# rare-resilience-ai/Osteosarcoma_DiffusionModel

Measured on AMD Instinct MI355X. Metric: synthetic patients/sec (full T-step reverse sample), higher is better.
Workload: dtype f32; 1 GPU; reverse sampling of conditional patients, T=1000, D=2000 (50 mut + 1900 expr + 50 pathway), hidden [256,512,256], 3 scenario conditions (BASELINE config 3); patients_per_gpu=100000, T=1000, parallelism=patients sharded over 1 GPU(s), no collective, sampler=chain, chunk_rows=65536, streams=2, graph=True

## Files before the change

osteosarcoma_diffusionmodel_amd/csrc/chain.h:

```cpp
#pragma once
#include "gemm_glds.h"
#include "epilogues.h"
#include "xpose.h"
#include "launch.h"

namespace osd {

constexpr int CHAIN_MAX_LAYERS = 24;
enum : int { CK_INPUT = 0, CK_GN32 = 1, CK_GN64 = 2, CK_POST = 3 };
enum : unsigned { CHAIN_OK = 0, CHAIN_TIMEOUT = 1, CHAIN_ABORT = 2 };

struct ChainLayer {
  const float* A; int lda;
  int K, K0;
  int F;
  int in0, ld0, in1, ld1;
  int out, ldo;
  int kind;
  const float* bias; const float* gamma; const float* beta;
};

struct ChainArgs {
  ChainLayer L[CHAIN_MAX_LAYERS];
  int n_layers;
  float* ws; long long ws_stride;
  float* x; int D;
  int n, n_tiles;
  int t_first, n_steps;
  unsigned base_done;
  const float* cproj; int ldc;
  const float* temb; int ldt;
  const float* coef;
  const float* z; int ldzz; long long z_step_stride; int z_t_first;
  uint64_t seed; uint32_t row_offset;
  float* mut_mask; int mutation_dim;
  unsigned* progress;
  unsigned* status;
  unsigned* queue;
  unsigned* cu_arrivals;
  int stagger;
  unsigned long long spin_budget;
  unsigned long long* stamps;
};

typedef __attribute__((address_space(1))) unsigned gu32;

__device__ __forceinline__ unsigned ld_relaxed_agent(const unsigned* p) {
  return __hip_atomic_load(p, __ATOMIC_RELAXED, __HIP_MEMORY_SCOPE_AGENT);
}
__device__ __forceinline__ void st_relaxed_agent(unsigned* p, unsigned v) {
  __hip_atomic_store(p, v, __ATOMIC_RELAXED, __HIP_MEMORY_SCOPE_AGENT);
}

__device__ __forceinline__ bool chain_wait(const unsigned* word, unsigned want, unsigned* status, unsigned long long budget, int lane) {
  if ((unsigned)__builtin_amdgcn_readfirstlane((int)ld_relaxed_agent(word)) >= want) return true;
  const unsigned long long t0 = __builtin_amdgcn_s_memrealtime();
  for (;;) {
    __builtin_amdgcn_s_sleep(32);
    if ((unsigned)__builtin_amdgcn_readfirstlane((int)ld_relaxed_agent(word)) >= want) return true;
    if ((unsigned)__builtin_amdgcn_readfirstlane((int)ld_relaxed_agent(status)) != CHAIN_OK) return false;
    if (__builtin_amdgcn_s_memrealtime() - t0 > budget) {
      if (lane == 0) st_relaxed_agent(status, CHAIN_TIMEOUT);
      return false;
    }
  }
}

constexpr int CHAIN_PRM_FLOATS = 512;

template <int NPB>
struct XposeRowsOut {
  const WaveXpose<NPB>& xp; float* out; int ldo;
  __device__ __forceinline__ void put(int fb, int pb, int q, int l31, int h, float4 v) const { (void)fb; xp.put(pb, q, l31, h, v); }
  __device__ __forceinline__ void flush(int fb, int lane) const { xp.template store_rows<false>(out + 32 * fb, ldo, lane, 0, 0); }
};
template <int NPB>
struct XposeRowsIn {
  const WaveXpose<NPB>& xp; const float* src; int ld;
  __device__ __forceinline__ void load(int fb, int lane) const { xp.template load_rows<false>(src + 32 * fb, ld, lane, 0, 0); }
  __device__ __forceinline__ float4 get(int fb, int pb, int q, int l31, int h) const { (void)fb; return xp.get(pb, q, l31, h); }
};

template <int GW, int NFB, int NPB, int PS, class Out>
__device__ __forceinline__ void chain_gn_silu(f32x16 (&acc)[NFB][NPB], const float* __restrict__ prm, int fl, const Out& o, int lane,
                                              unsigned long long* ts = nullptr) {
  static_assert(GW >= 8 && NFB * 32 >= GW, "wave must own whole groups");
  constexpr int RPG = GW / 2;
  constexpr int NG = NFB * 16 / RPG;
  const int l31 = lane & 31, h = lane >> 5;
#pragma unroll
  for (int fb = 0; fb < NFB; ++fb)
#pragma unroll
    for (int q = 0; q < 4; ++q) {
      const float4 bv = *reinterpret_cast<const float4*>(prm + fl + 32 * fb + 8 * q + 4 * h);
#pragma unroll
      for (int pb = 0; pb < NPB; ++pb) {
        acc[fb][pb][4 * q] += bv.x; acc[fb][pb][4 * q + 1] += bv.y;
        acc[fb][pb][4 * q + 2] += bv.z; acc[fb][pb][4 * q + 3] += bv.w;
      }
    }
  if (ts) { asm volatile("s_waitcnt vmcnt(0) lgkmcnt(0)" ::: "memory"); ts[0] = __builtin_amdgcn_s_memtime(); }
  float mean[NPB][NG], rstd[NPB][NG];
#pragma unroll
  for (int pb = 0; pb < NPB; ++pb)
#pragma unroll
    for (int g = 0; g < NG; ++g) {
      float s = 0.f;
#pragma unroll
      for (int j = 0; j < RPG; ++j) { const int Li = g * RPG + j; s += acc[Li / 16][pb][Li % 16]; }
      s += swap_halves(s);
      const float m = s * (1.0f / GW);
      float qs = 0.f;
#pragma unroll
      for (int j = 0; j < RPG; ++j) { const int Li = g * RPG + j; const float d = acc[Li / 16][pb][Li % 16] - m; qs = fmaf(d, d, qs); }
      qs += swap_halves(qs);
      mean[pb][g] = m;
      rstd[pb][g] = 1.0f / sqrtf(qs * (1.0f / GW) + GN_EPS);
    }
  if (ts) { asm volatile("s_nop 0" ::: "memory"); ts[1] = __builtin_amdgcn_s_memtime(); ts[2] = ts[1]; }
#pragma unroll
  for (int fb = 0; fb < NFB; ++fb) {
#pragma unroll
    for (int q = 0; q < 4; ++q) {
      const int f = fl + 32 * fb + 8 * q + 4 * h;
      const float4 gv = *reinterpret_cast<const float4*>(prm + PS + f);
      const float4 bev = *reinterpret_cast<const float4*>(prm + 2 * PS + f);
      const int g = (fb * 16 + 4 * q) / RPG;
#pragma unroll
      for (int pb = 0; pb < NPB; ++pb) {
        const float m = mean[pb][g], r = rstd[pb][g];
        float4 y;
        y.x = silu_f(fmaf((acc[fb][pb][4 * q] - m) * r, gv.x, bev.x));
        y.y = silu_f(fmaf((acc[fb][pb][4 * q + 1] - m) * r, gv.y, bev.y));
        y.z = silu_f(fmaf((acc[fb][pb][4 * q + 2] - m) * r, gv.z, bev.z));
        y.w = silu_f(fmaf((acc[fb][pb][4 * q + 3] - m) * r, gv.w, bev.w));
        o.put(fb, pb, q, l31, h, y);
      }
    }
    o.flush(fb, lane);
  }
}

template <int NFB, int NPB, int PS, class In, class Out>
__device__ __forceinline__ void chain_input(f32x16 (&acc)[NFB][NPB], const float* __restrict__ prm, int fl, const In& in, const Out& o, int lane) {
  const int l31 = lane & 31, h = lane >> 5;
#pragma unroll
  for (int fb = 0; fb < NFB; ++fb) {
    in.load(fb, lane);
#pragma unroll
    for (int q = 0; q < 4; ++q) {
      const int f = fl + 32 * fb + 8 * q + 4 * h;
      const float4 bv = *reinterpret_cast<const float4*>(prm + f);
      const float4 tv = *reinterpret_cast<const float4*>(prm + PS + f);
#pragma unroll
      for (int pb = 0; pb < NPB; ++pb) {
        const float4 cv = in.get(fb, pb, q, l31, h);
        float4 v;
        v.x = ((acc[fb][pb][4 * q] + bv.x) + tv.x) + cv.x;
        v.y = ((acc[fb][pb][4 * q + 1] + bv.y) + tv.y) + cv.y;
        v.z = ((acc[fb][pb][4 * q + 2] + bv.z) + tv.z) + cv.z;
        v.w = ((acc[fb][pb][4 * q + 3] + bv.w) + tv.w) + cv.w;
        o.put(fb, pb, q, l31, h, v);
      }
    }
    o.flush(fb, lane);
  }
}

#ifndef OSD_EXP
#define OSD_EXP 0
#endif
template <int NFB, int NPB, bool PRE = false, bool GUARD = true>
__device__ __forceinline__ void chain_posterior(f32x16 (&acc)[NFB][NPB], const float* __restrict__ prm, int fl, float* __restrict__ x, int ldx,
                                                int prow, int pcol, float cA, float cB, float cC, int t, const float* __restrict__ zrow, int ldzz,
                                                uint64_t seed, uint32_t row_id0, int f_glob, float* __restrict__ mut_mask, int mutation_dim,
                                                const WaveXpose<NPB>& xp, int lane, float4 (*pre)[4 * NPB] = nullptr) {
  const int l31 = lane & 31, h = lane >> 5;
  if (prow <= 0) return;
  const bool do_mask = t == 0 && mut_mask != nullptr;
#pragma unroll
  for (int fb = 0; fb < NFB; ++fb) {
    const int cols = pcol - 32 * fb;
    if (GUARD && cols <= 0) break;
    if constexpr (PRE) {
      if (!(OSD_EXP & 2)) {
        xp.commit_rows(*pre, lane);
        if (fb + 1 < NFB && cols - 32 > 0) xp.template issue_rows<GUARD>(*pre, x + 32 * (fb + 1), ldx, lane, prow, cols - 32);
      }
    } else {
      xp.template load_rows<GUARD>(x + 32 * fb, ldx, lane, prow, cols);
    }
#pragma unroll
    for (int pb = 0; pb < NPB; ++pb) {
      const int p = 32 * pb + l31;
      const int pc = (!GUARD || p < prow) ? p : prow - 1;
#pragma unroll
      for (int q = 0; q < 4; ++q) {
        const int fo = 32 * fb + 8 * q + 4 * h;
        const float4 bv = *reinterpret_cast<const float4*>(prm + fl + fo);
        const float e[4] = {acc[fb][pb][4 * q] + bv.x, acc[fb][pb][4 * q + 1] + bv.y, acc[fb][pb][4 * q + 2] + bv.z, acc[fb][pb][4 * q + 3] + bv.w};
        const float4 xq = xp.get(pb, q, l31, h);
        const float xv[4] = {xq.x, xq.y, xq.z, xq.w};
        float4 zz = make_float4(0.f, 0.f, 0.f, 0.f);
        if (t > 0 && cC != 0.f) {
          if (zrow) {
            const int fc = (!GUARD || fo < pcol - 4) ? fo : pcol - 4;
            zz = ldg4(zrow + (size_t)pc * ldzz + fc);
          } else if (!(OSD_EXP & 1)) {
            zz = randn4(seed, row_id0 + (uint32_t)p, (uint32_t)((f_glob + fo) >> 2), (uint32_t)t, TAG_POSTERIOR);
          }
        }
        const float zv[4] = {zz.x, zz.y, zz.z, zz.w};
        float o[4];
#pragma unroll
        for (int r = 0; r < 4; ++r) o[r] = fmaf(cA, xv[r], fmaf(cB, e[r], cC * zv[r]));
        if (do_mask && p < prow && fo < pcol && f_glob + fo < mutation_dim) {
          float* mrow = mut_mask + (size_t)p * mutation_dim;
#pragma unroll
          for (int r = 0; r < 4; ++r)
            if (f_glob + fo + r < mutation_dim) stg1(mrow + f_glob + fo + r, (o[r] > 0.5f) ? 1.0f : 0.0f);
        }
        xp.put(pb, q, l31, h, make_float4(o[0], o[1], o[2], o[3]));
      }
    }
    if (!(OSD_EXP & 4)) xp.template store_rows<GUARD>(x + 32 * fb, ldx, lane, prow, cols);
  }
}

#ifndef CHAIN_EPI_PRIO
#define CHAIN_EPI_PRIO 0
#endif
#ifndef CHAIN_BP
#define CHAIN_BP 128
#endif
#if CHAIN_BP == 128
typedef Tile<128, 128, 64, 64> ChainTile;
constexpr int CHAIN_WPS = 2;
#else
typedef Tile<128, 64, 64, 32> ChainTile;
constexpr int CHAIN_WPS = 3;
#endif
#ifdef OSD_DIAG
constexpr int CHAIN_KCNT = 12;
constexpr int CHAIN_STAMP_FLOATS = 2 * 4 * CHAIN_KCNT;
#else
constexpr int CHAIN_KCNT = 10;
constexpr int CHAIN_STAMP_FLOATS = 80;
#endif
constexpr int CHAIN_PRM_OFF = 2 * (ChainTile::BF * BK + ChainTile::BP * BK) + 4 + CHAIN_STAMP_FLOATS;
constexpr int CHAIN_LDS_BYTES = (CHAIN_PRM_OFF + 2 * CHAIN_PRM_FLOATS) * 4;
static_assert(CHAIN_PRM_OFF % 4 == 0, "parameter blocks are read as float4");

template <bool STAMP>
__global__ __launch_bounds__(NTHREADS, CHAIN_WPS) void chain_kernel(const ChainArgs* __restrict__ gp) {
  const ChainArgs& a = *gp;
  typedef ChainTile T;
  typedef GldsTile<T> G;
  static_assert(T::BF == 128 && T::BP % 32 == 0, "staging below assumes a 128-row weight image");
  constexpr int NW = NTHREADS / 64;
  constexpr int NPW = 16 / NW;
  constexpr int NPWB = T::BP / 8 / NW;
  constexpr int PROWS = 8 * NW;
  constexpr unsigned PBYTES = 1024u * NW;
  extern __shared__ __attribute__((aligned(16))) float smem[];
  float* As0 = smem;
  float* As1 = smem + G::A_ELEMS;
  float* Bs0 = smem + 2 * G::A_ELEMS;
  float* Bs1 = smem + 2 * G::A_ELEMS + G::B_ELEMS;
  volatile int& s_flag = *reinterpret_cast<volatile int*>(smem + 2 * (G::A_ELEMS + G::B_ELEMS));

  const int tid = threadIdx.x;
  const int lane = tid & 63;
  const int wave = __builtin_amdgcn_readfirstlane(tid >> 6);
  const int wf = (wave / T::NWP) * T::WF;
  const int wp = (wave % T::NWP) * T::WP;

  float* const ws = a.ws + (long long)blockIdx.x * a.ws_stride;
  WaveXpose<T::NPB> xp;
  {
    const int xo = wave * (T::NPB * 1024);
    xp.buf = xo < G::A_ELEMS ? As1 + xo : Bs1 + (xo - G::A_ELEMS);
  }
  float* const prm_base = smem + CHAIN_PRM_OFF;
  int pcur = 0;

  if (a.cu_arrivals && a.stagger > 0) {
    if (wave == 0) {
      const unsigned hw = __builtin_amdgcn_s_getreg(0xF804);
      const unsigned xcc = __builtin_amdgcn_s_getreg(0xF814) & 7;
      const unsigned key = (xcc << 8) | ((hw >> 8) & 0xFF);
      unsigned r = 0;
      if (lane == 0) r = atomicAdd(a.cu_arrivals + key, 1u);
      s_flag = __builtin_amdgcn_readfirstlane((int)(r & 1u));
    }
    __syncthreads();
    const int late = __builtin_amdgcn_readfirstlane(s_flag);
    __syncthreads();
    if (late) {
      const unsigned long long t0 = __builtin_amdgcn_s_memtime();
      while (__builtin_amdgcn_s_memtime() - t0 < (unsigned long long)a.stagger) __builtin_amdgcn_s_sleep(16);
    }
  }

  unsigned long long c_dep = 0, c_pro = 0, c_k = 0, c_epi = 0, c_units = 0;
  unsigned long long* const kcnt = reinterpret_cast<unsigned long long*>(smem + 2 * (G::A_ELEMS + G::B_ELEMS) + 4);
  if constexpr (STAMP) {
    if (tid < 4 * CHAIN_KCNT) kcnt[tid] = 0;
    __syncthreads();
  }
  const unsigned long long c_start = STAMP ? __builtin_amdgcn_s_memtime() : 0;
  const long long n_units = (long long)a.n_tiles * a.n_steps;
  int c_iter = 0;
  (void)c_iter;
  for (;;) {
    const unsigned long long td0 = STAMP ? __builtin_amdgcn_s_memtime() : 0;
#ifdef CHAIN_STATIC_UNITS
    static_assert(true, "");
    const long long u = (long long)blockIdx.x + (long long)c_iter * gridDim.x;
    ++c_iter;
#else
    if (wave == 0) {
      unsigned nu = 0;
      if (lane == 0) nu = atomicAdd(a.queue, 1u);
      s_flag = __builtin_amdgcn_readfirstlane((int)nu);
    }
    __syncthreads();
    const long long u = (unsigned)__builtin_amdgcn_readfirstlane(s_flag);
    __syncthreads();
#endif
    if (u >= n_units) break;
    const int tile = (int)(u % a.n_tiles);
    const int si = (int)(u / a.n_tiles);
    const int t = a.t_first - si;
    const int p0 = tile * T::BP;
    const int P = (a.n - p0 < T::BP) ? a.n - p0 : T::BP;

    if (wave == 0) {
      bool ok = (unsigned)__builtin_amdgcn_readfirstlane((int)ld_relaxed_agent(a.status)) == CHAIN_OK;
      if (ok && si > 0) {
        ok = chain_wait(a.progress + tile, a.base_done + (unsigned)si, a.status, a.spin_budget, lane);
        if (ok) __builtin_amdgcn_fence(__ATOMIC_ACQUIRE, "agent");
      }
      s_flag = ok ? 1 : 0;
      asm volatile("s_waitcnt vmcnt(0) lgkmcnt(0)" ::: "memory");
    }
    __syncthreads();
    const int go = __builtin_amdgcn_readfirstlane(s_flag);
    if (!go) return;
    if constexpr (STAMP) { c_dep += __builtin_amdgcn_s_memtime() - td0; ++c_units; }

    auto first_stage = [&](const ChainLayer& Lr, int f0n, bool do_a, bool do_b, int pb) {
      struct { const float* A; int lda, F, in0, ld0, K0, K; } Ln{Lr.A, Lr.lda, Lr.F, Lr.in0, Lr.ld0, Lr.K0, Lr.K};
      if (do_a && wave < 2) {
        const int kind = Lr.kind;
        const float* src = Lr.bias;
        if (wave == 1) src = Lr.beta;
        else if (lane >= 32) src = kind == CK_INPUT ? a.temb + (size_t)t * a.ldt : (kind == CK_POST ? Lr.bias : Lr.gamma);
        if (wave == 0 || (kind != CK_INPUT && kind != CK_POST)) {
          int f = f0n + 4 * (lane & 31);
          f = f < Ln.F - 4 ? f : Ln.F - 4;
          glds16(src + f, __builtin_amdgcn_readfirstlane(lds_addr(prm_base + pb * CHAIN_PRM_FLOATS) + (unsigned)wave * 1024u));
        }
      }
      const float* const xrows = a.x + (size_t)p0 * a.D;
      int ln = lane;
      asm volatile("" : "+v"(ln));
      const int r0 = wave * 8 + (ln >> 3);
      const int k4 = 4 * ((ln & 7) ^ ((r0 >> 1) & 7));
      const unsigned la = __builtin_amdgcn_readfirstlane(lds_addr(As0) + (unsigned)wave * 1024u);
      const unsigned lb = __builtin_amdgcn_readfirstlane(lds_addr(Bs0) + (unsigned)wave * 1024u);
      if (do_a) {
#pragma unroll
        for (int j = 0; j < NPW; ++j) {
          int rg = f0n + r0 + PROWS * j;
          rg = rg < Ln.F ? rg : Ln.F - 1;
          glds16(Ln.A + (size_t)rg * Ln.lda + k4, __builtin_amdgcn_readfirstlane(la + (unsigned)j * PBYTES));
        }
      }
      if (do_b) {
        const bool from_x = Ln.in0 < 0;
        const float* bb = from_x ? xrows : ws + Ln.in0;
        const int rows = from_x ? P : T::BP;
        const int kend = Ln.K0 < Ln.K ? Ln.K0 : Ln.K;
        const int k = k4 < kend - 4 ? k4 : kend - 4;
#pragma unroll
        for (int j = 0; j < NPWB; ++j) {
          int rg = r0 + PROWS * j;
          rg = rg < rows ? rg : rows - 1;
          glds16(bb + (size_t)rg * Ln.ld0 + k, __builtin_amdgcn_readfirstlane(lb + (unsigned)j * PBYTES));
        }
      }
    };
    unsigned long long tt0 = STAMP ? __builtin_amdgcn_s_memtime() : 0;
    first_stage(a.L[0], 0, true, true, pcur);
    asm volatile("s_waitcnt vmcnt(0)" ::: "memory");
    __syncthreads();

    for (int l = 0; l < a.n_layers; ++l) {
      const ChainLayer& L = a.L[l];
      const gfloat_ptr LA = uniform_ptr(L.A);
      const int Llda = L.lda, LK0 = L.K0, Lld0 = L.ld0, Lld1 = L.ld1;
      const int F = L.F, K = L.K;
      const float* const B0g = (L.in0 < 0) ? a.x + (size_t)p0 * a.D : ws + L.in0;
      const float* const B1g = ws + L.in1;
      const gfloat_ptr B0 = uniform_ptr(B0g), B1 = uniform_ptr(B1g);
      const int rowsB = (L.in0 < 0) ? P : T::BP;
      const int nk = (K + BK - 1) / BK;
      const int nft = (F + T::BF - 1) / T::BF;
      for (int ft = 0; ft < nft; ++ft) {
        const int f0 = ft * T::BF;
        int ln = lane;
        asm volatile("" : "+v"(ln));
        const int l31 = ln & 31, h = ln >> 5;
        int st_row[NPW], st_k4[NPW];
#pragma unroll
        for (int j = 0; j < NPW; ++j) {
          st_row[j] = (j * NW + wave) * 8 + (ln >> 3);
          st_k4[j] = 4 * ((ln & 7) ^ ((st_row[j] >> 1) & 7));
        }
        int a_rd[T::NFB], a_sw[T::NFB], b_rd[T::NPB], b_sw[T::NPB];
#pragma unroll
        for (int fb = 0; fb < T::NFB; ++fb) { const int R = wf + 32 * fb + l31; a_rd[fb] = R * BK; a_sw[fb] = h ^ ((R >> 1) & 7); }
#pragma unroll
        for (int pb = 0; pb < T::NPB; ++pb) { const int R = wp + 32 * pb + l31; b_rd[pb] = R * BK; b_sw[pb] = h ^ ((R >> 1) & 7); }
        unsigned offA[NPW], offB[NPWB];
#pragma unroll
        for (int j = 0; j < NPW; ++j) {
          int rg = f0 + st_row[j];
          rg = rg < F ? rg : F - 1;
          offA[j] = (unsigned)(rg * Llda + st_k4[j]) * 4u;
        }
#pragma unroll
        for (int j = 0; j < NPWB; ++j) {
          int rb = st_row[j];
          rb = rb < rowsB ? rb : rowsB - 1;
          offB[j] = (unsigned)(rb * Lld0 + st_k4[j]) * 4u;
        }
        int b_panel = 0;
        auto b_offsets_for = [&](int k0) {
          const int want = k0 < LK0 ? 0 : 1;
          if (want != b_panel) {
            b_panel = want;
            const int ld = want ? Lld1 : Lld0;
#pragma unroll
            for (int j = 0; j < NPWB; ++j) {
              int rb = st_row[j];
              rb = rb < rowsB ? rb : rowsB - 1;
              offB[j] = (unsigned)(rb * ld + st_k4[j]) * 4u;
            }
          }
        };
        struct StageCtx { gfloat_ptr sa, sb; unsigned la, lb; int k0; bool tail; };
        auto stage_begin = [&](int k0, float* As, float* Bs) {
          b_offsets_for(k0);
          const bool first = k0 < LK0;
          const int kend = first ? (LK0 < K ? LK0 : K) : K - LK0;
          const int kl = first ? k0 : k0 - LK0;
          StageCtx c;
          c.sa = LA + __builtin_amdgcn_readfirstlane(k0);
          c.sb = (first ? B0 : B1) + __builtin_amdgcn_readfirstlane(kl);
          c.la = __builtin_amdgcn_readfirstlane(lds_addr(As) + (unsigned)wave * 1024u);
          c.lb = __builtin_amdgcn_readfirstlane(lds_addr(Bs) + (unsigned)wave * 1024u);
          c.k0 = k0;
          c.tail = kl + BK > kend;
          return c;
        };
        auto piece = [&](const StageCtx& c, int j) {
          if (j < NPW) glds16s(c.sa, offA[j], __builtin_amdgcn_readfirstlane(c.la + (unsigned)j * PBYTES));
          else glds16s(c.sb, offB[j - NPW], __builtin_amdgcn_readfirstlane(c.lb + (unsigned)(j - NPW) * PBYTES));
        };
        auto stage_tail = [&](const StageCtx& c) {
#pragma unroll
          for (int j = 0; j < NPW; ++j) piece(c, j);
          const bool first = c.k0 < LK0;
          const int kend = first ? (LK0 < K ? LK0 : K) : K - LK0;
          const int kl = first ? c.k0 : c.k0 - LK0;
          const float* bb = first ? B0g : B1g;
          const int ld = first ? Lld0 : Lld1;
#pragma unroll
          for (int jb = 0; jb < NPWB; ++jb) {
            int k = kl + st_k4[jb];
            k = k < kend - 4 ? k : kend - 4;
            int rg = st_row[jb];
            rg = rg < rowsB ? rg : rowsB - 1;
            glds16(bb + (size_t)rg * ld + k, __builtin_amdgcn_readfirstlane(c.lb + (unsigned)jb * PBYTES));
          }
        };
        const unsigned long long tt1 = STAMP ? __builtin_amdgcn_s_memtime() : 0;

        unsigned long long c_kw = 0, c_kb = 0;
        (void)c_kw; (void)c_kb;
        f32x16 acc[T::NFB][T::NPB];
#pragma unroll
        for (int i = 0; i < T::NFB; ++i)
#pragma unroll
          for (int j = 0; j < T::NPB; ++j)
#pragma unroll
            for (int r = 0; r < 16; ++r) acc[i][j][r] = 0.f;

        float fa0[T::NFB][4], fb0[T::NPB][4], fa1[T::NFB][4], fb1[T::NPB][4];
        auto frags = [&](const float* Ac, const float* Bc, int i, float (&fa)[T::NFB][4], float (&fb)[T::NPB][4]) {
#pragma unroll
          for (int fb_ = 0; fb_ < T::NFB; ++fb_) {
            const float4 tq = *reinterpret_cast<const float4*>(&Ac[a_rd[fb_] + 4 * (a_sw[fb_] ^ (2 * i))]);
            fa[fb_][0] = tq.x; fa[fb_][1] = tq.y; fa[fb_][2] = tq.z; fa[fb_][3] = tq.w;
          }
#pragma unroll
          for (int pb = 0; pb < T::NPB; ++pb) {
            const float4 tq = *reinterpret_cast<const float4*>(&Bc[b_rd[pb] + 4 * (b_sw[pb] ^ (2 * i))]);
            fb[pb][0] = tq.x; fb[pb][1] = tq.y; fb[pb][2] = tq.z; fb[pb][3] = tq.w;
          }
        };
        auto quarter = [&](const float (&fa)[T::NFB][4], const float (&fb)[T::NPB][4]) {
#pragma unroll
          for (int e = 0; e < 4; ++e)
#pragma unroll
            for (int fb_ = 0; fb_ < T::NFB; ++fb_)
#pragma unroll
              for (int pb = 0; pb < T::NPB; ++pb)
                acc[fb_][pb] = __builtin_amdgcn_mfma_f32_32x32x2f32(fa[fb_][e], fb[pb][e], acc[fb_][pb], 0, 0, 0);
        };
        __builtin_amdgcn_sched_barrier(0);
        if (nk > 1) {
          const StageCtx c = stage_begin(BK, As1, Bs1);
          if (c.tail) stage_tail(c);
          else {
#pragma unroll
            for (int j = 0; j < NPW + NPWB; ++j) piece(c, j);
          }
        }
        frags(As0, Bs0, 0, fa0, fb0);
        __builtin_amdgcn_sched_barrier(0);
        for (int kt = 0; kt < nk; ++kt) {
          float* Ac = (kt & 1) ? As1 : As0;
          float* Bc = (kt & 1) ? Bs1 : Bs0;
          const float* An = (kt & 1) ? As0 : As1;
          const float* Bn = (kt & 1) ? Bs0 : Bs1;
          frags(Ac, Bc, 1, fa1, fb1);
          quarter(fa0, fb0);
          frags(Ac, Bc, 2, fa0, fb0);
          quarter(fa1, fb1);
          frags(Ac, Bc, 3, fa1, fb1);
          const bool ahead = kt + 2 < nk;
          StageCtx c{};
          if (ahead) c = stage_begin((kt + 2) * BK, Ac, Bc);
          const bool whole = ahead && !c.tail;
          quarter(fa0, fb0);
          __builtin_amdgcn_sched_barrier(0);
          const unsigned long long tw0 = STAMP ? __builtin_amdgcn_s_memtime() : 0;
          asm volatile("s_waitcnt vmcnt(0)" ::: "memory");
          const unsigned long long tw1 = STAMP ? __builtin_amdgcn_s_memtime() : 0;
          asm volatile("s_waitcnt lgkmcnt(0)" ::: "memory");
          __syncthreads();
          if constexpr (STAMP) { const unsigned long long tw2 = __builtin_amdgcn_s_memtime(); c_kw += tw1 - tw0; c_kb += tw2 - tw1; }
          __builtin_amdgcn_sched_barrier(0);
          if (ahead && c.tail) stage_tail(c);
          if (whole) {
#pragma unroll
            for (int j = 0; j < NPW + NPWB; ++j) piece(c, j);
          }
          if (kt + 1 < nk) frags(An, Bn, 0, fa0, fb0);
          __builtin_amdgcn_sched_barrier(0);
          quarter(fa1, fb1);
        }

        const unsigned long long tt2 = STAMP ? __builtin_amdgcn_s_memtime() : 0;
        const bool same_layer = ft + 1 < nft;
        const bool has_next = same_layer || l + 1 < a.n_layers;
        const int ln_next = same_layer ? l : l + 1;
        const int f0_next = same_layer ? f0 + T::BF : 0;
        const bool early_b = same_layer;
        if (has_next) first_stage(a.L[ln_next], f0_next, true, early_b, pcur ^ 1);
        const int fw = f0 + wf;
        const float* const prm = prm_base + pcur * CHAIN_PRM_FLOATS;
        pcur ^= 1;
        if (CHAIN_EPI_PRIO) __builtin_amdgcn_s_setprio(CHAIN_EPI_PRIO);
        const ChainArgs* ep = gp;
        asm volatile("" : "+s"(ep));
        const ChainArgs& e = *ep;
        unsigned long long ets[3] = {0, 0, 0};
        if (L.kind == CK_GN64) {
          const XposeRowsOut<T::NPB> o{xp, ws + L.out + (size_t)wp * L.ldo + fw, L.ldo};
          chain_gn_silu<64, T::NFB, T::NPB, 128>(acc, prm, wf, o, lane, STAMP ? ets : nullptr);
        } else if (L.kind == CK_GN32) {
          const XposeRowsOut<T::NPB> o{xp, ws + L.out + (size_t)wp * L.ldo + fw, L.ldo};
          chain_gn_silu<32, T::NFB, T::NPB, 128>(acc, prm, wf, o, lane, STAMP ? ets : nullptr);
        } else if (L.kind == CK_INPUT) {
          const XposeRowsIn<T::NPB> ci{xp, e.cproj + (size_t)(p0 + wp) * e.ldc + fw, e.ldc};
          const XposeRowsOut<T::NPB> o{xp, ws + L.out + (size_t)wp * L.ldo + fw, L.ldo};
          chain_input<T::NFB, T::NPB, 128>(acc, prm, wf, ci, o, lane);
        } else {
          const float* c = e.coef + 4 * t;
          const float cA = c[0], cB = c[1], cC = c[2];
          const float* zrow = e.z ? e.z + (long long)(e.z_t_first - t) * e.z_step_stride + (size_t)(p0 + wp) * e.ldzz + fw : nullptr;
          float* const mm = e.mut_mask ? e.mut_mask + (size_t)(p0 + wp) * e.mutation_dim : nullptr;
          chain_posterior<T::NFB, T::NPB>(acc, prm, wf, e.x + (size_t)(p0 + wp) * e.D + fw, e.D, P - wp, F - fw, cA, cB, cC, t, zrow, e.ldzz,
                                          e.seed, e.row_offset + (uint32_t)(p0 + wp), fw, mm, e.mutation_dim, xp, lane);
        }
        if (CHAIN_EPI_PRIO) __builtin_amdgcn_s_setprio(0);
        unsigned long long tt3 = 0, te1 = 0, te2 = 0, te3 = 0, te4 = 0;
        if constexpr (STAMP) te1 = __builtin_amdgcn_s_memtime();
        if (early_b) {
          if constexpr (STAMP) tt3 = __builtin_amdgcn_s_memtime();
          static_assert(4 * T::NFB * T::NPB == 16 || 4 * T::NFB * T::NPB == 8, "counted wait below is written for 16 or 8 stores");
          if (L.kind == CK_POST) asm volatile("s_waitcnt vmcnt(0)" ::: "memory");
          else if (4 * T::NFB * T::NPB == 16) asm volatile("s_waitcnt vmcnt(16)" ::: "memory");
          else asm volatile("s_waitcnt vmcnt(8)" ::: "memory");
          if constexpr (STAMP) te2 = __builtin_amdgcn_s_memtime();
          __syncthreads();
          if constexpr (STAMP) te3 = te4 = __builtin_amdgcn_s_memtime();
        } else {
          asm volatile("s_waitcnt vmcnt(0)" ::: "memory");
          if constexpr (STAMP) te2 = __builtin_amdgcn_s_memtime();
          __syncthreads();
          if constexpr (STAMP) tt3 = te3 = __builtin_amdgcn_s_memtime();
          if (has_next) {
            first_stage(a.L[ln_next], 0, false, true, 0);
            asm volatile("s_waitcnt vmcnt(0)" ::: "memory");
            __syncthreads();
          }
          if constexpr (STAMP) te4 = __builtin_amdgcn_s_memtime();
        }
        if constexpr (STAMP) {
          c_pro += tt1 - tt0; c_k += tt2 - tt1; c_epi += tt3 - tt2;
          tt0 = tt3;
          if (tid == 0) {
            unsigned long long* kc = kcnt + CHAIN_KCNT * L.kind;
            kc[0] += tt2 - tt1; kc[1] += te1 - tt2; kc[2] += te2 - te1; kc[3] += te3 - te2; kc[4] += te4 - te3; kc[5] += 1;
            if constexpr (CHAIN_KCNT >= 12) { kc[10] += c_kw; kc[11] += c_kb; }
            if (ets[0]) { kc[6] += ets[0] - tt2; kc[7] += ets[1] - ets[0]; kc[8] += ets[2] - ets[1]; kc[9] += te1 - ets[2]; }
          }
        }
      }
    }

    if (wave == 0) {
      __builtin_amdgcn_fence(__ATOMIC_RELEASE, "agent");
      asm volatile("s_waitcnt vmcnt(0)" ::: "memory");
      if (lane == 0) st_relaxed_agent(a.progress + tile, a.base_done + (unsigned)si + 1u);
    }
  }
  if (STAMP && a.stamps && tid == 0) {
    unsigned long long* o = a.stamps + (size_t)blockIdx.x * 64;
    o[0] = c_dep; o[1] = c_pro; o[2] = c_k; o[3] = c_epi; o[4] = __builtin_amdgcn_s_memtime() - c_start; o[5] = c_units;
    o[6] = __builtin_amdgcn_s_getreg(0xF804);
    o[7] = __builtin_amdgcn_s_getreg(0xF814) & 7;
    for (int i = 0; i < 4 * CHAIN_KCNT; ++i) o[8 + i] = kcnt[i];
  }
}

}
```

osteosarcoma_diffusionmodel_amd/csrc/xpose.h:

```cpp
#pragma once
#include "gemm_glds.h"

namespace osd {


__device__ __forceinline__ int xsw(int row) { return (row ^ (row >> 3)) & 7; }
template <int NPB>
struct WaveXpose {
  float* buf;
  __device__ __forceinline__ void put(int pb, int q, int l31, int h, float4 v) const {
    const int sw = h ^ xsw(l31);
    *reinterpret_cast<float4*>(buf + l31 * 32 + pb * 1024 + 4 * (sw ^ ((2 * q) ^ (4 * pb & 7)))) = v;
  }
  __device__ __forceinline__ float4 get(int pb, int q, int l31, int h) const {
    const int sw = h ^ xsw(l31);
    return *reinterpret_cast<const float4*>(buf + l31 * 32 + pb * 1024 + 4 * (sw ^ ((2 * q) ^ (4 * pb & 7))));
  }
  template <bool GUARD>
  __device__ __forceinline__ void store_rows(float* __restrict__ g, int ld, int lane, int rows, int cols) const {
    const int c = lane & 7, r = lane >> 3, cr = c ^ r;
#pragma unroll
    for (int i0 = 0; i0 < 4 * NPB; i0 += 4) {
      float4 v[4];
#pragma unroll
      for (int j = 0; j < 4; ++j) v[j] = *reinterpret_cast<const float4*>(buf + r * 32 + (i0 + j) * 256 + 4 * (cr ^ ((i0 + j) & 7)));
#pragma unroll
      for (int j = 0; j < 4; ++j) {
        const int row = 8 * (i0 + j) + r;
        if (!GUARD || (row < rows && 4 * c < cols)) stg4(g + (size_t)row * ld + 4 * c, v[j]);
      }
    }
  }
  template <bool GUARD>
  __device__ __forceinline__ void load_rows(const float* __restrict__ g, int ld, int lane, int rows, int cols) const {
    const int c = lane & 7, r = lane >> 3, cr = c ^ r;
    float4 v[4 * NPB];
#pragma unroll
    for (int i = 0; i < 4 * NPB; ++i) {
      int row = 8 * i + r;
      int cc = 4 * c;
      if (GUARD) { row = row < rows ? row : rows - 1; cc = cc < cols - 4 ? cc : cols - 4; }
      v[i] = ldg4(g + (size_t)row * ld + cc);
    }
#pragma unroll
    for (int i = 0; i < 4 * NPB; ++i) *reinterpret_cast<float4*>(buf + r * 32 + i * 256 + 4 * (cr ^ (i & 7))) = v[i];
  }
  template <bool GUARD>
  __device__ __forceinline__ void issue_rows(float4 (&v)[4 * NPB], const float* __restrict__ g, int ld, int lane, int rows, int cols) const {
    const int c = lane & 7, r = lane >> 3;
#pragma unroll
    for (int i = 0; i < 4 * NPB; ++i) {
      int row = 8 * i + r;
      int cc = 4 * c;
      if (GUARD) { row = row < rows ? row : rows - 1; cc = cc < cols - 4 ? cc : cols - 4; }
      v[i] = ldg4(g + (size_t)row * ld + cc);
    }
  }
  __device__ __forceinline__ void commit_rows(const float4 (&v)[4 * NPB], int lane) const {
    const int c = lane & 7, r = lane >> 3, cr = c ^ r;
#pragma unroll
    for (int i = 0; i < 4 * NPB; ++i) *reinterpret_cast<float4*>(buf + r * 32 + i * 256 + 4 * (cr ^ (i & 7))) = v[i];
  }
};

}
```

Before: 23310 patients/s.

## Prefetch epilogue side inputs via direct-to-LDS DMA during the last K step

For the 2x2 tile configuration, the input-layer conditioning rows and the posterior x rows are now fetched with global-to-LDS DMA issued at the end of the GEMM K loop instead of being loaded synchronously in the epilogue. Per-quarter counted vmcnt waits replace the full load-then-transpose, and the second feature block is prefetched as soon as the first block's LDS slots are freed. Kernel argument reads are routed through constant address-space pointers so they become scalar loads. This hides epilogue load latency behind compute, but relies on hand-counted waits that must match exactly the number of DMAs in flight, and a wrong count risks reading stale data.

```diff
diff --git a/osteosarcoma_diffusionmodel_amd/csrc/chain.h b/osteosarcoma_diffusionmodel_amd/csrc/chain.h
--- a/osteosarcoma_diffusionmodel_amd/csrc/chain.h
+++ b/osteosarcoma_diffusionmodel_amd/csrc/chain.h
@@ -3,6 +3,7 @@
 #include "epilogues.h"
 #include "xpose.h"
 #include "launch.h"
+#include <type_traits>
 
 namespace osd {
 
@@ -44,6 +45,9 @@
 };
 
 typedef __attribute__((address_space(1))) unsigned gu32;
+typedef const __attribute__((address_space(4))) ChainArgs* chain_cargs_ptr;
+typedef const __attribute__((address_space(4))) ChainLayer* chain_clayer_ptr;
+typedef const __attribute__((address_space(4))) float* cfloat_ptr;
 
 __device__ __forceinline__ unsigned ld_relaxed_agent(const unsigned* p) {
   return __hip_atomic_load(p, __ATOMIC_RELAXED, __HIP_MEMORY_SCOPE_AGENT);
@@ -80,6 +84,28 @@
   __device__ __forceinline__ void load(int fb, int lane) const { xp.template load_rows<false>(src + 32 * fb, ld, lane, 0, 0); }
   __device__ __forceinline__ float4 get(int fb, int pb, int q, int l31, int h) const { (void)fb; return xp.get(pb, q, l31, h); }
 };
+template <int NPB, bool GUARD>
+struct XposeRowsDma {
+  const WaveXpose<NPB>& xp; gfloat_ptr src; int ld, rows, cols;
+  template <int PB>
+  __device__ __forceinline__ void issue(int fb, int lane) const { xp.template dma_rows<GUARD, 4 * PB>(src + 32 * fb, ld, lane, rows, cols - 32 * fb); }
+  __device__ __forceinline__ float4 get(int fb, int pb, int q, int l31, int h) const { (void)fb; return xp.get(pb, q, l31, h); }
+};
+template <int N>
+__device__ __forceinline__ void vm_wait() { asm volatile("s_waitcnt vmcnt(%0)" ::"n"(N) : "memory"); }
+
+__device__ __forceinline__ void side_wait_first(int nfs) {
+  if (nfs == 9) vm_wait<13>();
+  else if (nfs == 8) vm_wait<12>();
+  else if (nfs == 5) vm_wait<9>();
+  else if (nfs == 4) vm_wait<8>();
+  else vm_wait<4>();
+}
+__device__ __forceinline__ void side_wait(int half, bool full, bool has_fb1) {
+  if (half == 1) { if (full) vm_wait<8>(); else if (has_fb1) vm_wait<4>(); else vm_wait<0>(); }
+  else if (half == 2) { if (full) vm_wait<12>(); else vm_wait<4>(); }
+  else { if (full) vm_wait<8>(); else vm_wait<0>(); }
+}
 
 template <int GW, int NFB, int NPB, int PS, class Out>
 __device__ __forceinline__ void chain_gn_silu(f32x16 (&acc)[NFB][NPB], const float* __restrict__ prm, int fl, const Out& o, int lane,
@@ -165,6 +191,36 @@
     }
     o.flush(fb, lane);
   }
+}
+
+template <int PS, class In>
+__device__ __forceinline__ void chain_input_dma(f32x16 (&acc)[2][2], const float* __restrict__ prm, int fl, const In& in, const WaveXpose<2>& xp,
+                                                float* __restrict__ out, int ldo, int lane, int nfs) {
+  const int l31 = lane & 31, h = lane >> 5;
+  auto half = [&](auto FB, auto PB) {
+    constexpr int fb = decltype(FB)::value, pb = decltype(PB)::value;
+    if (fb == 0 && pb == 0) side_wait_first(nfs);
+    else side_wait(2 * fb + pb, true, true);
+#pragma unroll
+    for (int q = 0; q < 4; ++q) {
+      const int f = fl + 32 * fb + 8 * q + 4 * h;
+      const float4 bv = *reinterpret_cast<const float4*>(prm + f);
+      const float4 tv = *reinterpret_cast<const float4*>(prm + PS + f);
+      const float4 cv = in.get(fb, pb, q, l31, h);
+      float4 v;
+      v.x = ((acc[fb][pb][4 * q] + bv.x) + tv.x) + cv.x;
+      v.y = ((acc[fb][pb][4 * q + 1] + bv.y) + tv.y) + cv.y;
+      v.z = ((acc[fb][pb][4 * q + 2] + bv.z) + tv.z) + cv.z;
+      v.w = ((acc[fb][pb][4 * q + 3] + bv.w) + tv.w) + cv.w;
+      xp.put(pb, q, l31, h, v);
+    }
+    xp.template store_rows4<false, 4 * pb>(out + 32 * fb, ldo, lane, 0, 0, [&]() {
+      if constexpr (fb == 0) in.template issue<pb>(1, lane);
+    });
+  };
+  typedef std::integral_constant<int, 0> I0;
+  typedef std::integral_constant<int, 1> I1;
+  half(I0{}, I0{}); half(I0{}, I1{}); half(I1{}, I0{}); half(I1{}, I1{});
 }
 
 #ifndef OSD_EXP
@@ -187,7 +243,7 @@
         xp.commit_rows(*pre, lane);
         if (fb + 1 < NFB && cols - 32 > 0) xp.template issue_rows<GUARD>(*pre, x + 32 * (fb + 1), ldx, lane, prow, cols - 32);
       }
-    } else {
+    } else if (!(OSD_EXP & 2)) {
       xp.template load_rows<GUARD>(x + 32 * fb, ldx, lane, prow, cols);
     }
 #pragma unroll
@@ -225,6 +281,82 @@
     }
     if (!(OSD_EXP & 4)) xp.template store_rows<GUARD>(x + 32 * fb, ldx, lane, prow, cols);
   }
+}
+
+template <int NFB, int NPB, bool GUARD, bool INJ>
+__device__ __forceinline__ void posterior_half(f32x16 (&acc)[NFB][NPB], const float* __restrict__ prm, int fl, int fb, int pb, int prow, int pcol,
+                                               float cA, float cB, float cC, int t, const float* __restrict__ zrow, int ldzz, uint64_t seed,
+                                               uint32_t row_id0, int f_glob, float* __restrict__ mut_mask, int mutation_dim, bool do_mask,
+                                               const WaveXpose<NPB>& xp, int l31, int h) {
+  const int p = 32 * pb + l31;
+  const int pc = (!GUARD || p < prow) ? p : prow - 1;
+#pragma unroll
+  for (int q = 0; q < 4; ++q) {
+    const int fo = 32 * fb + 8 * q + 4 * h;
+    const float4 bv = *reinterpret_cast<const float4*>(prm + fl + fo);
+    const float e[4] = {acc[fb][pb][4 * q] + bv.x, acc[fb][pb][4 * q + 1] + bv.y, acc[fb][pb][4 * q + 2] + bv.z, acc[fb][pb][4 * q + 3] + bv.w};
+    const float4 xq = xp.get(pb, q, l31, h);
+    const float xv[4] = {xq.x, xq.y, xq.z, xq.w};
+    float4 zz = make_float4(0.f, 0.f, 0.f, 0.f);
+    if (t > 0 && cC != 0.f) {
+      if (INJ) {
+        const int fc = (!GUARD || fo < pcol - 4) ? fo : pcol - 4;
+        zz = ldg4(zrow + (size_t)pc * ldzz + fc);
+      } else if (!(OSD_EXP & 1)) {
+        zz = randn4(seed, row_id0 + (uint32_t)p, (uint32_t)((f_glob + fo) >> 2), (uint32_t)t, TAG_POSTERIOR);
+      }
+    }
+    const float zv[4] = {zz.x, zz.y, zz.z, zz.w};
+    float o[4];
+#pragma unroll
+    for (int r = 0; r < 4; ++r) o[r] = fmaf(cA, xv[r], fmaf(cB, e[r], cC * zv[r]));
+    if (do_mask && p < prow && fo < pcol && f_glob + fo < mutation_dim) {
+      float* mrow = mut_mask + (size_t)p * mutation_dim;
+#pragma unroll
+      for (int r = 0; r < 4; ++r)
+        if (f_glob + fo + r < mutation_dim) stg1(mrow + f_glob + fo + r, (o[r] > 0.5f) ? 1.0f : 0.0f);
+    }
+    xp.put(pb, q, l31, h, make_float4(o[0], o[1], o[2], o[3]));
+  }
+}
+
+template <class In>
+__device__ __forceinline__ void chain_posterior_dma(f32x16 (&acc)[2][2], const float* __restrict__ prm, int fl, float* __restrict__ x, int ldx,
+                                                    int prow, int pcol, float cA, float cB, float cC, int t, const float* __restrict__ zrow,
+                                                    int ldzz, uint64_t seed, uint32_t row_id0, int f_glob, float* __restrict__ mut_mask,
+                                                    int mutation_dim, const WaveXpose<2>& xp, const In& in, int lane, int nfs, bool full) {
+  const int l31 = lane & 31, h = lane >> 5;
+  if (prow <= 0 || pcol <= 0) return;
+  const bool do_mask = t == 0 && mut_mask != nullptr;
+  const bool has_fb1 = pcol > 32;
+  auto half = [&](auto FB, auto PB, auto ZS) {
+    constexpr int fb = decltype(FB)::value, pb = decltype(PB)::value;
+    if (!(OSD_EXP & 2)) {
+      if (fb == 0 && pb == 0) side_wait_first(nfs);
+      else side_wait(2 * fb + pb, full, has_fb1);
+    }
+    posterior_half<2, 2, true, decltype(ZS)::value>(acc, prm, fl, fb, pb, prow, pcol, cA, cB, cC, t, zrow, ldzz, seed, row_id0, f_glob, mut_mask, mutation_dim, do_mask,
+                               xp, l31, h);
+    if (OSD_EXP & 4) {
+      asm volatile("s_waitcnt lgkmcnt(0)" ::: "memory");
+      if (fb == 0 && has_fb1 && !(OSD_EXP & 2)) in.template issue<pb>(1, lane);
+    } else {
+      xp.template store_rows4<true, 4 * pb>(x + 32 * fb, ldx, lane, prow, pcol - 32 * fb, [&]() {
+        if (fb == 0 && has_fb1 && !(OSD_EXP & 2)) in.template issue<pb>(1, lane);
+      });
+    }
+  };
+  typedef std::integral_constant<int, 0> I0;
+  typedef std::integral_constant<int, 1> I1;
+  auto walk = [&](auto ZS) {
+    half(I0{}, I0{}, ZS);
+    half(I0{}, I1{}, ZS);
+    if (!has_fb1) return;
+    half(I1{}, I0{}, ZS);
+    half(I1{}, I1{}, ZS);
+  };
+  if (zrow) walk(std::true_type{});
+  else walk(std::false_type{});
 }
 
 #ifndef CHAIN_EPI_PRIO
@@ -262,6 +394,7 @@
   constexpr int NPWB = T::BP / 8 / NW;
   constexpr int PROWS = 8 * NW;
   constexpr unsigned PBYTES = 1024u * NW;
+  constexpr bool SIDE_DMA = T::NFB == 2 && T::NPB == 2;
   extern __shared__ __attribute__((aligned(16))) float smem[];
   float* As0 = smem;
   float* As1 = smem + G::A_ELEMS;
@@ -349,20 +482,27 @@
     if (!go) return;
     if constexpr (STAMP) { c_dep += __builtin_amdgcn_s_memtime() - td0; ++c_units; }
 
-    auto first_stage = [&](const ChainLayer& Lr, int f0n, bool do_a, bool do_b, int pb) {
-      struct { const float* A; int lda, F, in0, ld0, K0, K; } Ln{Lr.A, Lr.lda, Lr.F, Lr.in0, Lr.ld0, Lr.K0, Lr.K};
+    auto first_stage = [&](const ChainLayer& Lr, int f0n, bool do_a, bool do_b, int pb) -> int {
+      int n_dma = 0;
+      const ChainLayer* lp = &Lr;
+      const ChainArgs* ap = gp;
+      asm volatile("" : "+s"(lp), "+s"(ap));
+      const chain_clayer_ptr Lc = (chain_clayer_ptr)(uintptr_t)lp;
+      const chain_cargs_ptr ac = (chain_cargs_ptr)(uintptr_t)ap;
+      struct { const float* A; int lda, F, in0, ld0, K0, K; } Ln{Lc->A, Lc->lda, Lc->F, Lc->in0, Lc->ld0, Lc->K0, Lc->K};
       if (do_a && wave < 2) {
-        const int kind = Lr.kind;
-        const float* src = Lr.bias;
-        if (wave == 1) src = Lr.beta;
-        else if (lane >= 32) src = kind == CK_INPUT ? a.temb + (size_t)t * a.ldt : (kind == CK_POST ? Lr.bias : Lr.gamma);
+        const int kind = Lc->kind;
+        const float* src = Lc->bias;
+        if (wave == 1) src = Lc->beta;
+        else if (lane >= 32) src = kind == CK_INPUT ? ac->temb + (size_t)t * ac->ldt : (kind == CK_POST ? Lc->bias : Lc->gamma);
         if (wave == 0 || (kind != CK_INPUT && kind != CK_POST)) {
           int f = f0n + 4 * (lane & 31);
           f = f < Ln.F - 4 ? f : Ln.F - 4;
           glds16(src + f, __builtin_amdgcn_readfirstlane(lds_addr(prm_base + pb * CHAIN_PRM_FLOATS) + (unsigned)wave * 1024u));
-        }
-      }
-      const float* const xrows = a.x + (size_t)p0 * a.D;
+          n_dma += 1;
+        }
+      }
+      const float* const xrows = ac->x + (size_t)p0 * ac->D;
       int ln = lane;
       asm volatile("" : "+v"(ln));
       const int r0 = wave * 8 + (ln >> 3);
@@ -376,6 +516,7 @@
           rg = rg < Ln.F ? rg : Ln.F - 1;
           glds16(Ln.A + (size_t)rg * Ln.lda + k4, __builtin_amdgcn_readfirstlane(la + (unsigned)j * PBYTES));
         }
+        n_dma += NPW;
       }
       if (do_b) {
         const bool from_x = Ln.in0 < 0;
@@ -389,7 +530,9 @@
           rg = rg < rows ? rg : rows - 1;
           glds16(bb + (size_t)rg * Ln.ld0 + k, __builtin_amdgcn_readfirstlane(lb + (unsigned)j * PBYTES));
         }
-      }
+        n_dma += NPWB;
+      }
+      return n_dma;
     };
     unsigned long long tt0 = STAMP ? __builtin_amdgcn_s_memtime() : 0;
     first_stage(a.L[0], 0, true, true, pcur);
@@ -400,7 +543,8 @@
       const ChainLayer& L = a.L[l];
       const gfloat_ptr LA = uniform_ptr(L.A);
       const int Llda = L.lda, LK0 = L.K0, Lld0 = L.ld0, Lld1 = L.ld1;
-      const int F = L.F, K = L.K;
+      const int F = L.F, K = L.K, kind = L.kind;
+      const bool side_dma = SIDE_DMA && !(OSD_EXP & 2) && (kind == CK_INPUT || kind == CK_POST);
       const float* const B0g = (L.in0 < 0) ? a.x + (size_t)p0 * a.D : ws + L.in0;
       const float* const B1g = ws + L.in1;
       const gfloat_ptr B0 = uniform_ptr(B0g), B1 = uniform_ptr(B1g);
@@ -484,6 +628,25 @@
             int rg = st_row[jb];
             rg = rg < rowsB ? rg : rowsB - 1;
             glds16(bb + (size_t)rg * ld + k, __builtin_amdgcn_readfirstlane(c.lb + (unsigned)jb * PBYTES));
+          }
+        };
+        auto side_request = [&]() {
+          if constexpr (SIDE_DMA) {
+            const ChainArgs* sg = gp;
+            asm volatile("" : "+s"(sg));
+            const chain_cargs_ptr sp = (chain_cargs_ptr)(uintptr_t)sg;
+            if (kind == CK_POST) {
+              const int prow = P - wp, pcol = F - (f0 + wf);
+              if (prow > 0 && pcol > 0) {
+                const XposeRowsDma<T::NPB, true> in{xp, uniform_ptr(sp->x + (size_t)(p0 + wp) * sp->D + f0 + wf), sp->D, prow, pcol};
+                in.template issue<0>(0, ln);
+                in.template issue<1>(0, ln);
+              }
+            } else {
+              const XposeRowsDma<T::NPB, false> in{xp, uniform_ptr(sp->cproj + (size_t)(p0 + wp) * sp->ldc + f0 + wf), sp->ldc, 0, 0};
+              in.template issue<0>(0, ln);
+              in.template issue<1>(0, ln);
+            }
           }
         };
         const unsigned long long tt1 = STAMP ? __builtin_amdgcn_s_memtime() : 0;
@@ -560,42 +723,68 @@
             for (int j = 0; j < NPW + NPWB; ++j) piece(c, j);
           }
           if (kt + 1 < nk) frags(An, Bn, 0, fa0, fb0);
+          else if (side_dma) side_request();
           __builtin_amdgcn_sched_barrier(0);
           quarter(fa1, fb1);
         }
 
         const unsigned long long tt2 = STAMP ? __builtin_amdgcn_s_memtime() : 0;
+        const ChainArgs* ep = gp;
+        asm volatile("" : "+s"(ep));
+        const ChainArgs& e = *ep;
+        const chain_cargs_ptr ec = (chain_cargs_ptr)(uintptr_t)ep;
         const bool same_layer = ft + 1 < nft;
-        const bool has_next = same_layer || l + 1 < a.n_layers;
+        const bool has_next = same_layer || l + 1 < ec->n_layers;
         const int ln_next = same_layer ? l : l + 1;
         const int f0_next = same_layer ? f0 + T::BF : 0;
         const bool early_b = same_layer;
-        if (has_next) first_stage(a.L[ln_next], f0_next, true, early_b, pcur ^ 1);
+        int nfs = 0;
+        if (has_next) nfs = first_stage(a.L[ln_next], f0_next, true, early_b, pcur ^ 1);
         const int fw = f0 + wf;
         const float* const prm = prm_base + pcur * CHAIN_PRM_FLOATS;
         pcur ^= 1;
         if (CHAIN_EPI_PRIO) __builtin_amdgcn_s_setprio(CHAIN_EPI_PRIO);
-        const ChainArgs* ep = gp;
-        asm volatile("" : "+s"(ep));
-        const ChainArgs& e = *ep;
         unsigned long long ets[3] = {0, 0, 0};
-        if (L.kind == CK_GN64) {
-          const XposeRowsOut<T::NPB> o{xp, ws + L.out + (size_t)wp * L.ldo + fw, L.ldo};
+        const chain_clayer_ptr Lc = &ec->L[l];
+        bool post_full = false;
+        if (kind == CK_GN64) {
+          const XposeRowsOut<T::NPB> o{xp, ws + Lc->out + (size_t)wp * Lc->ldo + fw, Lc->ldo};
           chain_gn_silu<64, T::NFB, T::NPB, 128>(acc, prm, wf, o, lane, STAMP ? ets : nullptr);
-        } else if (L.kind == CK_GN32) {
-          const XposeRowsOut<T::NPB> o{xp, ws + L.out + (size_t)wp * L.ldo + fw, L.ldo};
+        } else if (kind == CK_GN32) {
+          const XposeRowsOut<T::NPB> o{xp, ws + Lc->out + (size_t)wp * Lc->ldo + fw, Lc->ldo};
           chain_gn_silu<32, T::NFB, T::NPB, 128>(acc, prm, wf, o, lane, STAMP ? ets : nullptr);
-        } else if (L.kind == CK_INPUT) {
-          const XposeRowsIn<T::NPB> ci{xp, e.cproj + (size_t)(p0 + wp) * e.ldc + fw, e.ldc};
-          const XposeRowsOut<T::NPB> o{xp, ws + L.out + (size_t)wp * L.ldo + fw, L.ldo};
-          chain_input<T::NFB, T::NPB, 128>(acc, prm, wf, ci, o, lane);
+        } else if (kind == CK_INPUT) {
+          if constexpr (SIDE_DMA && !(OSD_EXP & 2)) {
+            const int ldc = ec->ldc, ldo = Lc->ldo;
+            const XposeRowsDma<T::NPB, false> ci{xp, uniform_ptr(ec->cproj + (size_t)(p0 + wp) * ldc + fw), ldc, 0, 0};
+            chain_input_dma<128>(acc, prm, wf, ci, xp, ws + Lc->out + (size_t)wp * ldo + fw, ldo, lane, nfs);
+          } else {
+            const XposeRowsIn<T::NPB> ci{xp, e.cproj + (size_t)(p0 + wp) * e.ldc + fw, e.ldc};
+            const XposeRowsOut<T::NPB> o{xp, ws + Lc->out + (size_t)wp * Lc->ldo + fw, Lc->ldo};
+            chain_input<T::NFB, T::NPB, 128>(acc, prm, wf, ci, o, lane);
+          }
         } else {
-          const float* c = e.coef + 4 * t;
-          const float cA = c[0], cB = c[1], cC = c[2];
-          const float* zrow = e.z ? e.z + (long long)(e.z_t_first - t) * e.z_step_stride + (size_t)(p0 + wp) * e.ldzz + fw : nullptr;
-          float* const mm = e.mut_mask ? e.mut_mask + (size_t)(p0 + wp) * e.mutation_dim : nullptr;
-          chain_posterior<T::NFB, T::NPB>(acc, prm, wf, e.x + (size_t)(p0 + wp) * e.D + fw, e.D, P - wp, F - fw, cA, cB, cC, t, zrow, e.ldzz,
-                                          e.seed, e.row_offset + (uint32_t)(p0 + wp), fw, mm, e.mutation_dim, xp, lane);
+          if constexpr (SIDE_DMA) {
+            const cfloat_ptr c = (cfloat_ptr)(uintptr_t)(ec->coef + 4 * t);
+            const float cA = c[0], cB = c[1], cC = c[2];
+            const float* const z = ec->z;
+            const int ldzz = ec->ldzz, D = ec->D, mdim = ec->mutation_dim;
+            const float* zrow = z ? z + (long long)(ec->z_t_first - t) * ec->z_step_stride + (size_t)(p0 + wp) * ldzz + fw : nullptr;
+            float* const mask = ec->mut_mask;
+            float* const mm = mask ? mask + (size_t)(p0 + wp) * mdim : nullptr;
+            float* const xw = ec->x + (size_t)(p0 + wp) * D + fw;
+            const XposeRowsDma<T::NPB, true> xi{xp, uniform_ptr(xw), D, P - wp, F - fw};
+            post_full = P - wp >= T::WP && F - fw >= T::WF && !(t == 0 && mm) && !(OSD_EXP & 4);
+            chain_posterior_dma(acc, prm, wf, xw, D, P - wp, F - fw, cA, cB, cC, t, zrow, ldzz, ec->seed, ec->row_offset + (uint32_t)(p0 + wp), fw,
+                                mm, mdim, xp, xi, lane, nfs, post_full);
+          } else {
+            const float* c = e.coef + 4 * t;
+            const float cA = c[0], cB = c[1], cC = c[2];
+            const float* zrow = e.z ? e.z + (long long)(e.z_t_first - t) * e.z_step_stride + (size_t)(p0 + wp) * e.ldzz + fw : nullptr;
+            float* const mm = e.mut_mask ? e.mut_mask + (size_t)(p0 + wp) * e.mutation_dim : nullptr;
+            chain_posterior<T::NFB, T::NPB>(acc, prm, wf, e.x + (size_t)(p0 + wp) * e.D + fw, e.D, P - wp, F - fw, cA, cB, cC, t, zrow, e.ldzz,
+                                            e.seed, e.row_offset + (uint32_t)(p0 + wp), fw, mm, e.mutation_dim, xp, lane);
+          }
         }
         if (CHAIN_EPI_PRIO) __builtin_amdgcn_s_setprio(0);
         unsigned long long tt3 = 0, te1 = 0, te2 = 0, te3 = 0, te4 = 0;
@@ -603,7 +792,8 @@
         if (early_b) {
           if constexpr (STAMP) tt3 = __builtin_amdgcn_s_memtime();
           static_assert(4 * T::NFB * T::NPB == 16 || 4 * T::NFB * T::NPB == 8, "counted wait below is written for 16 or 8 stores");
-          if (L.kind == CK_POST) asm volatile("s_waitcnt vmcnt(0)" ::: "memory");
+          static_assert(!SIDE_DMA || 4 * T::NFB * T::NPB == 16, "post_full stands for sixteen stores");
+          if (kind == CK_POST && !post_full) asm volatile("s_waitcnt vmcnt(0)" ::: "memory");
           else if (4 * T::NFB * T::NPB == 16) asm volatile("s_waitcnt vmcnt(16)" ::: "memory");
           else asm volatile("s_waitcnt vmcnt(8)" ::: "memory");
           if constexpr (STAMP) te2 = __builtin_amdgcn_s_memtime();
@@ -625,7 +815,7 @@
           c_pro += tt1 - tt0; c_k += tt2 - tt1; c_epi += tt3 - tt2;
           tt0 = tt3;
           if (tid == 0) {
-            unsigned long long* kc = kcnt + CHAIN_KCNT * L.kind;
+            unsigned long long* kc = kcnt + CHAIN_KCNT * kind;
             kc[0] += tt2 - tt1; kc[1] += te1 - tt2; kc[2] += te2 - te1; kc[3] += te3 - te2; kc[4] += te4 - te3; kc[5] += 1;
             if constexpr (CHAIN_KCNT >= 12) { kc[10] += c_kw; kc[11] += c_kb; }
             if (ets[0]) { kc[6] += ets[0] - tt2; kc[7] += ets[1] - ets[0]; kc[8] += ets[2] - ets[1]; kc[9] += te1 - ets[2]; }
diff --git a/osteosarcoma_diffusionmodel_amd/csrc/xpose.h b/osteosarcoma_diffusionmodel_amd/csrc/xpose.h
--- a/osteosarcoma_diffusionmodel_amd/csrc/xpose.h
+++ b/osteosarcoma_diffusionmodel_amd/csrc/xpose.h
@@ -29,6 +29,33 @@
         const int row = 8 * (i0 + j) + r;
         if (!GUARD || (row < rows && 4 * c < cols)) stg4(g + (size_t)row * ld + 4 * c, v[j]);
       }
+    }
+  }
+  template <bool GUARD, int I0, class Freed>
+  __device__ __forceinline__ void store_rows4(float* __restrict__ g, int ld, int lane, int rows, int cols, const Freed& freed) const {
+    const int c = lane & 7, r = lane >> 3, cr = c ^ r;
+    float4 v[4];
+#pragma unroll
+    for (int j = 0; j < 4; ++j) v[j] = *reinterpret_cast<const float4*>(buf + r * 32 + (I0 + j) * 256 + 4 * (cr ^ ((I0 + j) & 7)));
+    asm volatile("s_waitcnt lgkmcnt(0)" ::: "memory");
+    freed();
+#pragma unroll
+    for (int j = 0; j < 4; ++j) {
+      const int row = 8 * (I0 + j) + r;
+      if (!GUARD || (row < rows && 4 * c < cols)) stg4(g + (size_t)row * ld + 4 * c, v[j]);
+    }
+  }
+  template <bool GUARD, int I0>
+  __device__ __forceinline__ void dma_rows(gfloat_ptr g, int ld, int lane, int rows, int cols) const {
+    const int s = lane & 7, r = lane >> 3, sr = s ^ r;
+    const unsigned dst = lds_addr(buf);
+#pragma unroll
+    for (int j = 0; j < 4; ++j) {
+      const int i = I0 + j;
+      int row = 8 * i + r;
+      int cc = 4 * (sr ^ (i & 7));
+      if (GUARD) { row = row < rows ? row : rows - 1; cc = cc < cols - 4 ? cc : cols - 4; }
+      glds16s(g, (unsigned)(row * ld + cc) * 4u, __builtin_amdgcn_readfirstlane(dst + 1024u * (unsigned)i));
     }
   }
   template <bool GUARD>
```

Measured after the change: 23500 patients/s (median of 6 runs). Within noise of the previous version (+0.8%).
